# lachinov/brats2019

Hardware: AMD Instinct MI355X
Metric: volumes_per_sec_fwd_bwd_128cubed_x4ch (higher is better)
Workload: dtype bf16

## Files before the change

brats2019_amd/csrc/pointwise.hip:

```cpp
#include "pw_helpers.hpp"
#include "augment_voxel.hpp"

namespace ru {

template <int VEC, int COT>
__global__ __launch_bounds__(256) void conv1_kernel(const Conv1Args a) {
    const int n = blockIdx.z;
    const int co0 = blockIdx.y * COT;
    const size_t V = a.V;
    const size_t v = ((size_t)blockIdx.x * 256 + threadIdx.x) * VEC;
    if (v >= V) return;
    float acc[COT][VEC];
#pragma unroll
    for (int o = 0; o < COT; ++o)
#pragma unroll
        for (int k = 0; k < VEC; ++k) acc[o][k] = 0.f;
    int widx[COT];
#pragma unroll
    for (int o = 0; o < COT; ++o) widx[o] = (co0 + o < a.Cout) ? co0 + o : a.Cout - 1;

    const float* xp = a.x0 + (size_t)n * a.C0 * V + v;
    const float* wr = a.wT;
#pragma unroll 4
    for (int c = 0; c < a.C0; ++c) {
// ... 466 lines not shown
        if (dbeta) dbeta[g * cpg + j] = (float)db;
    }
}
int gn_bwd_finalize_launch(const float* partials, int nblk, const float* gamma, const float* mean, const float* rstd,
                           float* coef, float* dgamma, float* dbeta, int N, int C, size_t V, int G, hipStream_t s, int s2_sign) {
    RU_REQUIRE(C % G == 0 && C / G <= 256, "groupnorm: C must be divisible by G (and C/G <= 256)");
    const size_t shm = (size_t)N * (C / G) * 2 * sizeof(double);
    RU_REQUIRE(shm <= 60000, "groupnorm backward: batch x channels-per-group too large for the finalize kernel");
    if (nblk > 32) hipLaunchKernelGGL(gn_bwd_finalize_kernel<64>, dim3(G), dim3(N * (C / G) > 4 ? 512 : 256), shm, s, partials, nblk, gamma, mean, rstd, coef, dgamma, dbeta, N, C, V, G, s2_sign);
    else if (nblk > 4) hipLaunchKernelGGL(gn_bwd_finalize_kernel<16>, dim3(G), dim3(256), shm, s, partials, nblk, gamma, mean, rstd, coef, dgamma, dbeta, N, C, V, G, s2_sign);
    else hipLaunchKernelGGL(gn_bwd_finalize_kernel<4>, dim3(G), dim3(256), shm, s, partials, nblk, gamma, mean, rstd, coef, dgamma, dbeta, N, C, V, G, s2_sign);
    RU_CHECK_LAUNCH("gn_bwd_finalize_kernel");
    return RU_OK;
}

template <int VEC>
__global__ __launch_bounds__(256) void gn_bwd_apply_kernel(const float* __restrict__ x, const float* __restrict__ dy, const float* __restrict__ scale,
                                                           const float* __restrict__ shift, const float* __restrict__ coef, float slope,
                                                           float* __restrict__ dx, size_t V) {
    const size_t row = blockIdx.y;
    const float a = scale[row], b = shift[row];
    const float cA = coef[row * 3], cB = coef[row * 3 + 1], cC = coef[row * 3 + 2];
    const size_t base = row * V;
    for (size_t v = ((size_t)blockIdx.x * 256 + threadIdx.x) * VEC; v < V; v += (size_t)gridDim.x * 256 * VEC) {
        if (VEC == 4) {
            const float4 t = *reinterpret_cast<const float4*>(x + base + v);
            const float4 d = *reinterpret_cast<const float4*>(dy + base + v);
            float4 o;
            o.x = cA * ((t.x * a + b) > 0.f ? d.x : d.x * slope) + (cB * t.x + cC);
            o.y = cA * ((t.y * a + b) > 0.f ? d.y : d.y * slope) + (cB * t.y + cC);
            o.z = cA * ((t.z * a + b) > 0.f ? d.z : d.z * slope) + (cB * t.z + cC);
            o.w = cA * ((t.w * a + b) > 0.f ? d.w : d.w * slope) + (cB * t.w + cC);
            *reinterpret_cast<float4*>(dx + base + v) = o;
        } else {
            const float t = x[base + v], d = dy[base + v];
            dx[base + v] = cA * ((t * a + b) > 0.f ? d : d * slope) + (cB * t + cC);
        }
    }
}
int gn_bwd_apply_launch(const float* x, const float* dy, const float* scale, const float* shift, const float* coef,
                        float slope, float* dx, int N, int C, size_t V, hipStream_t s) {
    if (V % 4 == 0) hipLaunchKernelGGL(gn_bwd_apply_kernel<4>, rows_grid(V, 4, N * C), dim3(256), 0, s, x, dy, scale, shift, coef, slope, dx, V);
    else hipLaunchKernelGGL(gn_bwd_apply_kernel<1>, rows_grid(V, 1, N * C), dim3(256), 0, s, x, dy, scale, shift, coef, slope, dx, V);
    RU_CHECK_LAUNCH("gn_bwd_apply_kernel");
    return RU_OK;
}

enum { EW_LRELU = 0, EW_LRELU_BWD = 1, EW_SIGMOID = 2, EW_SIGMOID_BWD = 3, EW_ADD = 4, EW_FILL = 5 };
template <int OP>
__global__ __launch_bounds__(256) void ew_kernel(const float* __restrict__ a, const float* __restrict__ b, float* __restrict__ y, size_t n, float p) {
    const size_t stride = (size_t)gridDim.x * 256;
    for (size_t i = (size_t)blockIdx.x * 256 + threadIdx.x; i < n; i += stride) {
        float r;
        if (OP == EW_LRELU) r = lrelu(a[i], p);
        else if (OP == EW_LRELU_BWD) r = a[i] > 0.f ? b[i] : b[i] * p;
        else if (OP == EW_SIGMOID) r = 1.f / (1.f + expf(-a[i]));
        else if (OP == EW_SIGMOID_BWD) { const float q = a[i]; r = b[i] * q * (1.f - q); }
        else if (OP == EW_ADD) r = a[i] + b[i];
        else r = p;
        y[i] = r;
    }
}
template <int OP>
static int ew_launch(const float* a, const float* b, float* y, size_t n, float p, hipStream_t s, const char* name) {
    if (n == 0) return RU_OK;
    hipLaunchKernelGGL(ew_kernel<OP>, dim3(grid1d(n, 256 * 4, 8192)), dim3(256), 0, s, a, b, y, n, p);
    RU_CHECK_LAUNCH(name);
    return RU_OK;
}
int lrelu_fwd_launch(const float* x, float* y, size_t n, float slope, hipStream_t s) { return ew_launch<EW_LRELU>(x, nullptr, y, n, slope, s, "lrelu"); }
int lrelu_bwd_launch(const float* yv, const float* dy, float* dx, size_t n, float slope, hipStream_t s) { return ew_launch<EW_LRELU_BWD>(yv, dy, dx, n, slope, s, "lrelu_bwd"); }
int sigmoid_launch(const float* x, float* y, size_t n, hipStream_t s) { return ew_launch<EW_SIGMOID>(x, nullptr, y, n, 0.f, s, "sigmoid"); }
int sigmoid_bwd_launch(const float* p, const float* dp, float* dz, size_t n, hipStream_t s) { return ew_launch<EW_SIGMOID_BWD>(p, dp, dz, n, 0.f, s, "sigmoid_bwd"); }
int add_launch(const float* a, const float* b, float* y, size_t n, hipStream_t s) { return ew_launch<EW_ADD>(a, b, y, n, 0.f, s, "add"); }
__global__ __launch_bounds__(256) void sum_partials_kernel(const float* __restrict__ part, int ksplit, size_t n, float* __restrict__ y) {
    const size_t n4 = n >> 2;
    for (size_t i = (size_t)blockIdx.x * 256 + threadIdx.x; i < n4; i += (size_t)gridDim.x * 256) {
        float4 acc = reinterpret_cast<const float4*>(part)[i];
        for (int z = 1; z < ksplit; ++z) {
            const float4 t = reinterpret_cast<const float4*>(part + (size_t)z * n)[i];
            acc.x += t.x; acc.y += t.y; acc.z += t.z; acc.w += t.w;
        }
        reinterpret_cast<float4*>(y)[i] = acc;
    }
    if (blockIdx.x == 0 && threadIdx.x < (n & 3)) {
        const size_t i = (n4 << 2) + threadIdx.x;
        float acc = part[i];
        for (int z = 1; z < ksplit; ++z) acc += part[(size_t)z * n + i];
        y[i] = acc;
    }
}
int sum_partials_launch(const float* part, int ksplit, size_t n, float* y, hipStream_t s) {
    RU_REQUIRE(part && y && ksplit >= 1, "sum_partials: bad argument");
    RU_REQUIRE(ksplit == 1 || (n & 3) == 0, "sum_partials: partial tensors of %zu floats are not 16-byte aligned to each other", n);
    hipLaunchKernelGGL(sum_partials_kernel, dim3(grid1d(n, 256 * 4, 2048)), dim3(256), 0, s, part, ksplit, n, y);
    RU_CHECK_LAUNCH("sum_partials_kernel");
    return RU_OK;
}
int fill_launch(float* p, float v, size_t n, hipStream_t s) { return ew_launch<EW_FILL>(nullptr, nullptr, p, n, v, s, "fill"); }

__global__ __launch_bounds__(256) void up2_fwd_kernel(const float* __restrict__ x, float* __restrict__ y, int NC, int D, int H, int W) {
    const int Do = 2 * D, Ho = 2 * H;
    const size_t total = (size_t)NC * Do * Ho * W;
    for (size_t i = (size_t)blockIdx.x * 256 + threadIdx.x; i < total; i += (size_t)gridDim.x * 256) {
        const int k = (int)(i % W);
        size_t r = i / W;
        const int yo = (int)(r % Ho); r /= Ho;
        const int zo = (int)(r % Do);
        const size_t nc = r / Do;
        int z0, z1, y0, y1; float lz0, lz1, ly0, ly1;
        up2_src(zo, D, z0, z1, lz0, lz1);
        up2_src(yo, H, y0, y1, ly0, ly1);
        const int km = k > 0 ? k - 1 : 0, kp = k < W - 1 ? k + 1 : k;
        const float* p00 = x + ((nc * D + z0) * H + y0) * (size_t)W;
        const float* p01 = x + ((nc * D + z0) * H + y1) * (size_t)W;
        const float* p10 = x + ((nc * D + z1) * H + y0) * (size_t)W;
        const float* p11 = x + ((nc * D + z1) * H + y1) * (size_t)W;
        const float e0 = k > 0 ? 0.25f : 1.f, e1 = k > 0 ? 0.75f : 0.f;
        const int ei0 = k > 0 ? km : 0, ei1 = k > 0 ? k : (W > 1 ? 1 : 0);
        const float ev = lz0 * (ly0 * (e0 * p00[ei0] + e1 * p00[ei1]) + ly1 * (e0 * p01[ei0] + e1 * p01[ei1])) +
                         lz1 * (ly0 * (e0 * p10[ei0] + e1 * p10[ei1]) + ly1 * (e0 * p11[ei0] + e1 * p11[ei1]));
        const float ov = lz0 * (ly0 * (0.75f * p00[k] + 0.25f * p00[kp]) + ly1 * (0.75f * p01[k] + 0.25f * p01[kp])) +
                         lz1 * (ly0 * (0.75f * p10[k] + 0.25f * p10[kp]) + ly1 * (0.75f * p11[k] + 0.25f * p11[kp]));
        float* yp = y + ((nc * Do + zo) * Ho + yo) * (size_t)(2 * W) + 2 * k;
        *reinterpret_cast<float2*>(yp) = make_float2(ev, ov);
    }
}
__global__ __launch_bounds__(256) void up2_fwd_vec_kernel(const float* __restrict__ x, float* __restrict__ y, int NC, int D, int H, int W) {
    const int Do = 2 * D, Ho = 2 * H, Wh = W / 2;
    const size_t total = (size_t)NC * Do * Ho * Wh;
    for (size_t i = (size_t)blockIdx.x * 256 + threadIdx.x; i < total; i += (size_t)gridDim.x * 256) {
        const int m = (int)(i % Wh);
        size_t r = i / Wh;
        const int yo = (int)(r % Ho); r /= Ho;
        const int zo = (int)(r % Do);
        const size_t nc = r / Do;
        int z0, z1, y0, y1; float lz0, lz1, ly0, ly1;
        up2_src(zo, D, z0, z1, lz0, lz1);
        up2_src(yo, H, y0, y1, ly0, ly1);
        const int k = 2 * m;
        const int km = k > 0 ? k - 1 : 0, kpp = k + 2 < W ? k + 2 : W - 1;
        const float* rows[4] = {x + ((nc * D + z0) * H + y0) * (size_t)W, x + ((nc * D + z0) * H + y1) * (size_t)W,
                                x + ((nc * D + z1) * H + y0) * (size_t)W, x + ((nc * D + z1) * H + y1) * (size_t)W};
        const float wgt[4] = {lz0 * ly0, lz0 * ly1, lz1 * ly0, lz1 * ly1};
        float o[4];
        float rowv[4][4];
#pragma unroll
        for (int q = 0; q < 4; ++q) {
            const float a0 = rows[q][km], a1 = rows[q][k], a2 = rows[q][k + 1], a3 = rows[q][kpp];
            rowv[q][0] = k > 0 ? 0.25f * a0 + 0.75f * a1 : 1.f * a1 + 0.f * a2;
            rowv[q][1] = 0.75f * a1 + 0.25f * a2;
            rowv[q][2] = 0.25f * a1 + 0.75f * a2;
            rowv[q][3] = 0.75f * a2 + 0.25f * a3;
        }
        (void)wgt;
#pragma unroll
        for (int t = 0; t < 4; ++t)
            o[t] = lz0 * (ly0 * rowv[0][t] + ly1 * rowv[1][t]) + lz1 * (ly0 * rowv[2][t] + ly1 * rowv[3][t]);
        *reinterpret_cast<float4*>(y + ((nc * Do + zo) * Ho + yo) * (size_t)(2 * W) + 4 * m) = make_float4(o[0], o[1], o[2], o[3]);
    }
}
int up2_fwd_launch(const float* x, float* y, int N, int C, int D, int H, int W, hipStream_t s) {
    if ((W & 1) == 0) {
        const size_t total = (size_t)N * C * 2 * D * 2 * H * (W / 2);
        hipLaunchKernelGGL(up2_fwd_vec_kernel, dim3(grid1d(total, 256)), dim3(256), 0, s, x, y, N * C, D, H, W);
        RU_CHECK_LAUNCH("up2_fwd_vec_kernel");
        return RU_OK;
    }
    const size_t total = (size_t)N * C * 2 * D * 2 * H * W;
    hipLaunchKernelGGL(up2_fwd_kernel, dim3(grid1d(total, 256)), dim3(256), 0, s, x, y, N * C, D, H, W);
    RU_CHECK_LAUNCH("up2_fwd_kernel");
    return RU_OK;
}

__global__ __launch_bounds__(256) void up2_bwd_kernel(const float* __restrict__ dy, float* __restrict__ dx, int NC, int D, int H, int W) {
    const int Do = 2 * D, Ho = 2 * H, Wo = 2 * W;
    const size_t total = (size_t)NC * D * H * W;
    for (size_t i = (size_t)blockIdx.x * 256 + threadIdx.x; i < total; i += (size_t)gridDim.x * 256) {
        const int kx = (int)(i % W);
        size_t r = i / W;
        const int ky = (int)(r % H); r /= H;
        const int kz = (int)(r % D);
        const size_t nc = r / D;
        float wz[4], wy[4], wx[4];
#pragma unroll
        for (int t = 0; t < 4; ++t) {
            const int oz = 2 * kz - 1 + t, oy = 2 * ky - 1 + t, ox = 2 * kx - 1 + t;
            wz[t] = (oz >= 0 && oz < Do) ? up2_coef(oz, D, kz) : 0.f;
            wy[t] = (oy >= 0 && oy < Ho) ? up2_coef(oy, H, ky) : 0.f;
            wx[t] = (ox >= 0 && ox < Wo) ? up2_coef(ox, W, kx) : 0.f;
        }
        float acc = 0.f;
#pragma unroll
        for (int a = 0; a < 4; ++a) {
            if (wz[a] == 0.f) continue;
            const int oz = 2 * kz - 1 + a;
            float accy = 0.f;
#pragma unroll
            for (int b = 0; b < 4; ++b) {
                if (wy[b] == 0.f) continue;
                const int oy = 2 * ky - 1 + b;
                const float* p = dy + ((nc * Do + oz) * Ho + oy) * (size_t)Wo;
                float accx = 0.f;
#pragma unroll
                for (int c = 0; c < 4; ++c) {
                    const int ox = 2 * kx - 1 + c;
                    if (wx[c] != 0.f) accx += wx[c] * p[ox];
                }
                accy += wy[b] * accx;
            }
            acc += wz[a] * accy;
        }
        dx[i] = acc;
    }
}
__global__ __launch_bounds__(256) void up2_bwd_vec_kernel(const float* __restrict__ dy, float* __restrict__ dx, int NC, int D, int H, int W) {
    const int Do = 2 * D, Ho = 2 * H, Wo = 2 * W, Wh = W / 2;
    const size_t total = (size_t)NC * D * H * Wh;
    for (size_t i = (size_t)blockIdx.x * 256 + threadIdx.x; i < total; i += (size_t)gridDim.x * 256) {
        const int m = (int)(i % Wh);
        size_t r = i / Wh;
        const int ky = (int)(r % H); r /= H;
        const int kz = (int)(r % D);
        const size_t nc = r / D;
        const int k0 = 2 * m, k1 = 2 * m + 1;
        float wz[4], wy[4], wa[4], wb[4];
#pragma unroll
        for (int t = 0; t < 4; ++t) {
            const int oz = 2 * kz - 1 + t, oy = 2 * ky - 1 + t, oa = 2 * k0 - 1 + t, ob = 2 * k1 - 1 + t;
            wz[t] = (oz >= 0 && oz < Do) ? up2_coef(oz, D, kz) : 0.f;
            wy[t] = (oy >= 0 && oy < Ho) ? up2_coef(oy, H, ky) : 0.f;
            wa[t] = (oa >= 0 && oa < Wo) ? up2_coef(oa, W, k0) : 0.f;
            wb[t] = (ob >= 0 && ob < Wo) ? up2_coef(ob, W, k1) : 0.f;
        }
        const int oxl = 4 * m - 1 >= 0 ? 4 * m - 1 : 0, oxr = 4 * m + 4 < Wo ? 4 * m + 4 : Wo - 1;
        float acc0 = 0.f, acc1 = 0.f;
#pragma unroll
        for (int a = 0; a < 4; ++a) {
            const int oz = 2 * kz - 1 + a;
            const int ozc = oz < 0 ? 0 : (oz >= Do ? Do - 1 : oz);
            float ay0 = 0.f, ay1 = 0.f;
#pragma unroll
            for (int b = 0; b < 4; ++b) {
                const int oy = 2 * ky - 1 + b;
                const int oyc = oy < 0 ? 0 : (oy >= Ho ? Ho - 1 : oy);
                const float* p = dy + ((nc * Do + ozc) * Ho + oyc) * (size_t)Wo;
                const float4 f = *reinterpret_cast<const float4*>(p + 4 * m);
                const float fl = p[oxl], fr = p[oxr];
                ay0 += wy[b] * (wa[0] * fl + wa[1] * f.x + wa[2] * f.y + wa[3] * f.z);
                ay1 += wy[b] * (wb[0] * f.y + wb[1] * f.z + wb[2] * f.w + wb[3] * fr);
            }
            acc0 += wz[a] * ay0;
            acc1 += wz[a] * ay1;
        }
        *reinterpret_cast<float2*>(dx + ((nc * D + kz) * H + ky) * (size_t)W + 2 * m) = make_float2(acc0, acc1);
    }
}
int up2_bwd_launch(const float* dy, float* dx, int N, int C, int D, int H, int W, hipStream_t s) {
    if ((W & 1) == 0) {
        const size_t tv = (size_t)N * C * D * H * (W / 2);
        hipLaunchKernelGGL(up2_bwd_vec_kernel, dim3(grid1d(tv, 256)), dim3(256), 0, s, dy, dx, N * C, D, H, W);
        RU_CHECK_LAUNCH("up2_bwd_vec_kernel");
        return RU_OK;
    }
    const size_t total = (size_t)N * C * D * H * W;
    hipLaunchKernelGGL(up2_bwd_kernel, dim3(grid1d(total, 256)), dim3(256), 0, s, dy, dx, N * C, D, H, W);
    RU_CHECK_LAUNCH("up2_bwd_kernel");
    return RU_OK;
}

constexpr int BG_CHUNK = 16384;
size_t bias_grad_workspace_bytes(int N, int C, size_t V) { return (size_t)N * C * ((V + BG_CHUNK - 1) / BG_CHUNK) * sizeof(float); }
__global__ __launch_bounds__(256) void bias_partial_kernel(const float* __restrict__ dy, float* __restrict__ part, size_t V, int nblk) {
    __shared__ float buf[4];
    const size_t row = blockIdx.y;
    const size_t v0 = (size_t)blockIdx.x * BG_CHUNK;
    const size_t v1 = v0 + BG_CHUNK < V ? v0 + BG_CHUNK : V;
    float s1 = 0.f;
    for (size_t v = v0 + threadIdx.x; v < v1; v += 256) s1 += dy[row * V + v];
    s1 = block_sum(s1, buf);
    if (threadIdx.x == 0) part[row * nblk + blockIdx.x] = s1;
}
__global__ __launch_bounds__(256) void bias_final_kernel(const float* __restrict__ part, float* __restrict__ db, int N, int C, int nblk) {
    __shared__ double buf[4];
    const int c = blockIdx.x;
    double s1 = 0.0;
    for (int i = threadIdx.x; i < N * nblk; i += 256) {
        const int n = i / nblk, b = i % nblk;
        s1 += (double)part[((size_t)n * C + c) * nblk + b];
    }
    s1 = block_sum_d(s1, buf);
    if (threadIdx.x == 0) db[c] = (float)s1;
}
int bias_grad_launch(const float* dy, float* db, int N, int C, size_t V, void* ws, size_t ws_bytes, hipStream_t s) {
    if (!ws || ws_bytes < bias_grad_workspace_bytes(N, C, V)) { set_error("bias_grad: workspace too small"); return RU_ENOMEM; }
    const int nblk = (int)((V + BG_CHUNK - 1) / BG_CHUNK);
    hipLaunchKernelGGL(bias_partial_kernel, dim3(nblk, N * C), dim3(256), 0, s, dy, (float*)ws, V, nblk);
    RU_CHECK_LAUNCH("bias_partial_kernel");
    hipLaunchKernelGGL(bias_final_kernel, dim3(C), dim3(256), 0, s, (const float*)ws, db, N, C, nblk);
    RU_CHECK_LAUNCH("bias_final_kernel");
    return RU_OK;
}

template <bool CRIT>
__global__ __launch_bounds__(256) void head_grad_c4_kernel(const float* __restrict__ p, const float* __restrict__ dp, float* __restrict__ d4,
                                                           float* __restrict__ part, int C, size_t V, int nblk, const CritGradArgs cg) {
    __shared__ float buf[4];
    const size_t n = blockIdx.y;
    const size_t v0 = (size_t)blockIdx.x * BG_CHUNK;
    const size_t v1 = v0 + BG_CHUNK < V ? v0 + BG_CHUNK : V;
    const float* pp = p + n * C * V;
    const float* dpp = dp + n * C * V;
    float4* op = reinterpret_cast<float4*>(d4) + n * V;
    float sum[4] = {0.f, 0.f, 0.f, 0.f};
    float kg[4] = {0.f, 0.f, 0.f, 0.f}, kp[4] = {0.f, 0.f, 0.f, 0.f}, cb = 0.f;
    const float one_eps = (float)(1.0 + 1e-6);
    if constexpr (CRIT) {
        for (int c = 0; c < C && c < 4; ++c) {
            const double I = cg.sums[c] + 1e-6, U = cg.sums[C + c] + 2e-6;
            const double k = (double)cg.priority * (2.0 / (double)C) * (double)cg.w_dice;
            kg[c] = (float)(-k / U);
            kp[c] = (float)(2.0 * k * I / (U * U));
        }
        cb = (float)((double)cg.w_bce / cg.count);
    }
    for (size_t v = v0 + (size_t)threadIdx.x * 4; v < v1; v += 1024) {
        float d[4][4];
#pragma unroll
        for (int c = 0; c < 4; ++c) {
            const bool ok = c < C;
            const float4 q = *reinterpret_cast<const float4*>(pp + (ok ? c : 0) * V + v);
            float4 g = *reinterpret_cast<const float4*>(dpp + (ok ? c : 0) * V + v);
            if constexpr (CRIT) {
                const float pv[4] = {q.x, q.y, q.z, q.w}, gv[4] = {g.x, g.y, g.z, g.w};
                float o[4];
#pragma unroll
                for (int e = 0; e < 4; ++e) o[e] = crit_grad_value(pv[e], gv[e], kg[c], kp[c], cb, cg.bgw, one_eps);
                g = make_float4(o[0], o[1], o[2], o[3]);
            }
            d[c][0] = ok ? g.x * q.x * (1.f - q.x) : 0.f;
            d[c][1] = ok ? g.y * q.y * (1.f - q.y) : 0.f;
            d[c][2] = ok ? g.z * q.z * (1.f - q.z) : 0.f;
            d[c][3] = ok ? g.w * q.w * (1.f - q.w) : 0.f;
            sum[c] += (d[c][0] + d[c][1]) + (d[c][2] + d[c][3]);
        }
#pragma unroll
        for (int e = 0; e < 4; ++e) op[v + e] = make_float4(d[0][e], d[1][e], d[2][e], d[3][e]);
    }
#pragma unroll
    for (int c = 0; c < 4; ++c) {
        const float t = block_sum(sum[c], buf);
        if (threadIdx.x == 0 && c < C) part[(n * C + c) * nblk + blockIdx.x] = t;
    }
}
int head_grad_c4_launch(const float* p, const float* dp, float* d4, float* db, int N, int C, size_t V, void* ws, size_t ws_bytes, hipStream_t s) {
    RU_REQUIRE(C > 0 && C <= 4 && V % 4 == 0, "head_grad_c4: 1..4 channels, V %% 4 == 0");
    if (!ws || ws_bytes < bias_grad_workspace_bytes(N, C, V)) { set_error("head_grad_c4: workspace too small"); return RU_ENOMEM; }
    const int nblk = (int)((V + BG_CHUNK - 1) / BG_CHUNK);
    hipLaunchKernelGGL(head_grad_c4_kernel<false>, dim3(nblk, N), dim3(256), 0, s, p, dp, d4, (float*)ws, C, V, nblk, CritGradArgs{});
    RU_CHECK_LAUNCH("head_grad_c4_kernel");
    hipLaunchKernelGGL(bias_final_kernel, dim3(C), dim3(256), 0, s, (const float*)ws, db, N, C, nblk);
    RU_CHECK_LAUNCH("bias_final_kernel");
    return RU_OK;
}
int head_grad_c4_crit_launch(const float* p, const CritGradArgs& cg, float* d4, float* db, int N, int C, size_t V, void* ws, size_t ws_bytes, hipStream_t s) {
    RU_REQUIRE(C > 0 && C <= 4 && V % 4 == 0 && cg.target && cg.sums, "head_grad_c4_crit: 1..4 channels, V %% 4 == 0, target and sums");
    if (!ws || ws_bytes < bias_grad_workspace_bytes(N, C, V)) { set_error("head_grad_c4_crit: workspace too small"); return RU_ENOMEM; }
    const int nblk = (int)((V + BG_CHUNK - 1) / BG_CHUNK);
    hipLaunchKernelGGL(head_grad_c4_kernel<true>, dim3(nblk, N), dim3(256), 0, s, p, cg.target, d4, (float*)ws, C, V, nblk, cg);
    RU_CHECK_LAUNCH("head_grad_c4_kernel<crit>");
    hipLaunchKernelGGL(bias_final_kernel, dim3(C), dim3(256), 0, s, (const float*)ws, db, N, C, nblk);
    RU_CHECK_LAUNCH("bias_final_kernel");
    return RU_OK;
}

constexpr int CR_CHUNK = 8192;
int crit_tiles(size_t V) { return (int)((V + CR_CHUNK - 1) / CR_CHUNK); }
__global__ __launch_bounds__(256) void crit_partial_kernel(const float* __restrict__ p, const float* __restrict__ g, float* __restrict__ part,
                                                           size_t V, int nblk, float bgw) {
    __shared__ float buf[4];
    const size_t row = blockIdx.y;
    const size_t v0 = (size_t)blockIdx.x * CR_CHUNK;
    const size_t v1 = v0 + CR_CHUNK < V ? v0 + CR_CHUNK : V;
    const float one_eps = (float)(1.0 + 1e-6);
    float si = 0.f, su = 0.f, sb = 0.f;
    for (size_t v = v0 + threadIdx.x; v < v1; v += 256) {
        const float pv = p[row * V + v], gv = g[row * V + v];
        si += pv * gv;
        su += pv * pv + gv;
        sb += gv * logf(pv + 1e-6f) + bgw * (1.f - gv) * logf(one_eps - pv);
    }
    si = block_sum(si, buf);
    su = block_sum(su, buf);
    sb = block_sum(sb, buf);
    if (threadIdx.x == 0) {
        float* q = part + (row * nblk + blockIdx.x) * 3;
        q[0] = si; q[1] = su; q[2] = sb;
    }
}
__global__ __launch_bounds__(256) void crit_final_kernel(const float* __restrict__ part, double* __restrict__ sums, int N, int C, int nblk) {
    __shared__ double buf[4];
    double bce = 0.0;
    for (int c = 0; c < C; ++c) {
        double si = 0.0, su = 0.0, sb = 0.0;
        for (int i = threadIdx.x; i < N * nblk; i += 256) {
            const int n = i / nblk, b = i % nblk;
            const float* q = part + (((size_t)n * C + c) * nblk + b) * 3;
            si += (double)q[0]; su += (double)q[1]; sb += (double)q[2];
        }
        si = block_sum_d(si, buf);
        su = block_sum_d(su, buf);
        sb = block_sum_d(sb, buf);
        if (threadIdx.x == 0) { sums[c] = si; sums[C + c] = su; }
        bce += sb;
    }
    if (threadIdx.x == 0) sums[2 * C] = bce;
}
int crit_sums_launch(const float* p, const float* g, double* sums, int N, int C, size_t V, float bgw, void* ws, size_t ws_bytes, hipStream_t s) {
    const int nblk = crit_tiles(V);
    if (!ws || ws_bytes < (size_t)N * C * nblk * 3 * sizeof(float)) { set_error("criterion: workspace too small"); return RU_ENOMEM; }
    hipLaunchKernelGGL(crit_partial_kernel, dim3(nblk, N * C), dim3(256), 0, s, p, g, (float*)ws, V, nblk, bgw);
    RU_CHECK_LAUNCH("crit_partial_kernel");
    hipLaunchKernelGGL(crit_final_kernel, dim3(1), dim3(256), 0, s, (const float*)ws, sums, N, C, nblk);
    RU_CHECK_LAUNCH("crit_final_kernel");
    return RU_OK;
}
__global__ void crit_value_kernel(const double* __restrict__ sums, int C, double count, double priority, double w_dice, double w_bce,
                                  double* __restrict__ out) {
    double q = threadIdx.x < (unsigned)C ? 2.0 * (sums[threadIdx.x] + 1e-6) / (sums[C + threadIdx.x] + 2e-6) : 0.0;
    for (int o = 32; o > 0; o >>= 1) q += __shfl_xor(q, o);
    if (threadIdx.x == 0) {
        const double dice = priority * (1.0 - q / C), bce = -sums[2 * C] / count;
        out[0] = w_dice * dice + w_bce * bce; out[1] = dice; out[2] = bce;
    }
}
int crit_value_launch(const double* sums, int C, double count, double priority, double w_dice, double w_bce, double* out3, hipStream_t s) {
    hipLaunchKernelGGL(crit_value_kernel, dim3(1), dim3(64), 0, s, sums, C, count, priority, w_dice, w_bce, out3);
    RU_CHECK_LAUNCH("crit_value_kernel");
    return RU_OK;
}
__global__ __launch_bounds__(256) void crit_grad_kernel(const float* __restrict__ p, const float* __restrict__ g, const double* __restrict__ sums,
                                                        double count, float w_dice, float w_bce, float bgw, float priority,
                                                        float* __restrict__ dp, int C, size_t V) {
    const size_t row = blockIdx.y;
    const int c = (int)(row % C);
    const double I = sums[c] + 1e-6, U = sums[C + c] + 2e-6;
    const double k = (double)priority * (2.0 / (double)C) * (double)w_dice;
    const float cg = (float)(-k / U), cp = (float)(2.0 * k * I / (U * U));
    const float cb = (float)((double)w_bce / count);
    const float one_eps = (float)(1.0 + 1e-6);
    for (size_t v = (size_t)blockIdx.x * 256 + threadIdx.x; v < V; v += (size_t)gridDim.x * 256) {
        const float pv = p[row * V + v], gv = g[row * V + v];
        dp[row * V + v] = crit_grad_value(pv, gv, cg, cp, cb, bgw, one_eps);
    }
}
int crit_grad_launch(const float* p, const float* g, const double* sums, double count, float w_dice, float w_bce,
                     float bgw, float priority, float* dp, int N, int C, size_t V, hipStream_t s) {
    hipLaunchKernelGGL(crit_grad_kernel, rows_grid(V, 1, N * C), dim3(256), 0, s, p, g, sums, count, w_dice, w_bce, bgw, priority, dp, C, V);
    RU_CHECK_LAUNCH("crit_grad_kernel");
    return RU_OK;
}

__global__ __launch_bounds__(256) void tta_merge_kernel(const float* __restrict__ p, int K, unsigned flips, float* __restrict__ mean_out,
                                                        unsigned char* __restrict__ mask_out, unsigned long long* __restrict__ counts,
                                                        int C, int D, int H, int W) {
    __shared__ unsigned int cnt[4];
    const size_t V = (size_t)D * H * W;
    const int c = blockIdx.y;
    if (threadIdx.x < 4) cnt[threadIdx.x] = 0;
    __syncthreads();
    unsigned int local = 0;
    for (size_t v = (size_t)blockIdx.x * 256 + threadIdx.x; v < V; v += (size_t)gridDim.x * 256) {
        const int x = (int)(v % W);
        const int y = (int)((v / W) % H);
        const int z = (int)(v / ((size_t)W * H));
        float acc = 0.f;
        for (int k = 0; k < K; ++k) {
            const unsigned f = (flips >> (3 * k)) & 7u;
            const int zz = (f & 1u) ? D - 1 - z : z, yy = (f & 2u) ? H - 1 - y : y, xx = (f & 4u) ? W - 1 - x : x;
            const float t = p[(((size_t)k * C + c) * D + zz) * H * W + (size_t)yy * W + xx];
            acc = k == 0 ? t : acc + t;
        }
        const float m = acc / (float)K;
        if (mean_out) mean_out[(size_t)c * V + v] = m;
        const bool on = m > 0.5f;
        mask_out[(size_t)c * V + v] = on ? 1 : 0;
        local += on ? 1u : 0u;
    }
    atomicAdd(&cnt[threadIdx.x >> 6], local);
    __syncthreads();
    if (threadIdx.x == 0) atomicAdd(&counts[c], (unsigned long long)cnt[0] + cnt[1] + cnt[2] + cnt[3]);
}
__global__ __launch_bounds__(256) void compose_labels_kernel(const unsigned char* __restrict__ mask, const unsigned long long* __restrict__ counts,
                                                             unsigned long long et_min, unsigned char* __restrict__ labels, size_t V) {
    const bool et_on = counts[2] > et_min;
    for (size_t v = (size_t)blockIdx.x * 256 + threadIdx.x; v < V; v += (size_t)gridDim.x * 256) {
        unsigned char l = 0;
        if (mask[v]) l = 2;
        if (mask[V + v]) l = 1;
        if (et_on && mask[2 * V + v]) l = 4;
        labels[v] = l;
    }
}
int tta_merge_launch(const float* p, int K, unsigned flips, float* mean_out, unsigned char* mask, unsigned long long* counts, int C, int D, int H, int W, hipStream_t s) {
    RU_REQUIRE(K >= 1 && K <= 8 && C >= 1, "tta_merge: 1..8 predictions");
    hipError_t e = hipMemsetAsync(counts, 0, sizeof(unsigned long long) * C, s);
    if (e != hipSuccess) return hip_fail(e, "hipMemsetAsync(counts)");
    const size_t V = (size_t)D * H * W;
    hipLaunchKernelGGL(tta_merge_kernel, dim3(grid1d(V, 256 * 8, 512), C), dim3(256), 0, s, p, K, flips, mean_out, mask, counts, C, D, H, W);
    RU_CHECK_LAUNCH("tta_merge_kernel");
    return RU_OK;
}
int compose_labels_launch(const unsigned char* mask, const unsigned long long* counts, unsigned long long et_min, unsigned char* labels, size_t V, hipStream_t s) {
    hipLaunchKernelGGL(compose_labels_kernel, dim3(grid1d(V, 256, 4096)), dim3(256), 0, s, mask, counts, et_min, labels, V);
    RU_CHECK_LAUNCH("compose_labels_kernel");
    return RU_OK;
}

__global__ __launch_bounds__(256) void layout_convert_kernel(const float* __restrict__ src, float* __restrict__ dst, int CB, size_t V, int to_c16) {
    __shared__ float tile[16][65];
    const size_t v0 = (size_t)blockIdx.x * 64;
    const size_t nb = blockIdx.y;
    const int t = threadIdx.x;
    const float* s_nc = src + nb * 16 * V;
    float* d_nc = dst + nb * 16 * V;
    if (to_c16) {
#pragma unroll
        for (int j = 0; j < 4; ++j) {
            const int c = (t >> 6) + 4 * j, v = t & 63;
            tile[c][v] = v0 + v < V ? s_nc[(size_t)c * V + v0 + v] : 0.f;
        }
        __syncthreads();
#pragma unroll
        for (int j = 0; j < 4; ++j) {
            const int e = t + 256 * j, v = e >> 4, c = e & 15;
            if (v0 + v < V) d_nc[(v0 + v) * 16 + c] = tile[c][v];
        }
    } else {
#pragma unroll
        for (int j = 0; j < 4; ++j) {
            const int e = t + 256 * j, v = e >> 4, c = e & 15;
            tile[c][v] = v0 + v < V ? s_nc[(v0 + v) * 16 + c] : 0.f;
        }
        __syncthreads();
#pragma unroll
        for (int j = 0; j < 4; ++j) {
            const int c = (t >> 6) + 4 * j, v = t & 63;
            if (v0 + v < V) d_nc[(size_t)c * V + v0 + v] = tile[c][v];
        }
    }
}
int layout_convert_launch(const float* src, float* dst, int N, int C, size_t V, int to_c16, hipStream_t s) {
    RU_REQUIRE(C > 0 && C % 16 == 0, "layout_convert: C must be a multiple of 16");
    hipLaunchKernelGGL(layout_convert_kernel, dim3((unsigned)((V + 63) / 64), (unsigned)(N * (C / 16))), dim3(256), 0, s, src, dst, C / 16, V, to_c16);
    RU_CHECK_LAUNCH("layout_convert_kernel");
    return RU_OK;
}

__global__ __launch_bounds__(256) void pad_to_c16_kernel(const float* __restrict__ src, float* __restrict__ dst, int C, size_t V) {
    const size_t n = blockIdx.y;
    const float* sp = src + n * C * V;
    float4* dp = reinterpret_cast<float4*>(dst + n * 16 * V);
    for (size_t f = (size_t)blockIdx.x * 256 + threadIdx.x; f < V * 4; f += (size_t)gridDim.x * 256) {
        const size_t v = f >> 2;
        const int c0 = (int)(f & 3) * 4;
        float4 o;
        o.x = c0 + 0 < C ? sp[(size_t)(c0 + 0) * V + v] : 0.f;
        o.y = c0 + 1 < C ? sp[(size_t)(c0 + 1) * V + v] : 0.f;
        o.z = c0 + 2 < C ? sp[(size_t)(c0 + 2) * V + v] : 0.f;
        o.w = c0 + 3 < C ? sp[(size_t)(c0 + 3) * V + v] : 0.f;
        dp[f] = o;
    }
}
int pad_to_c16_launch(const float* src, float* dst, int N, int C, size_t V, hipStream_t s) {
    RU_REQUIRE(C > 0 && C <= 16, "pad_to_c16: 1..16 channels");
    hipLaunchKernelGGL(pad_to_c16_kernel, dim3(grid1d(V * 4, 256, 4096), (unsigned)N), dim3(256), 0, s, src, dst, C, V);
    RU_CHECK_LAUNCH("pad_to_c16_kernel");
    return RU_OK;
}

__global__ __launch_bounds__(256) void pad_to_c4_kernel(const float* __restrict__ src, float* __restrict__ dst, int C, size_t V) {
    const size_t n = blockIdx.y;
    const float* sp = src + n * C * V;
    float4* dp = reinterpret_cast<float4*>(dst) + n * V;
    for (size_t v = (size_t)blockIdx.x * 256 + threadIdx.x; v < V; v += (size_t)gridDim.x * 256) {
        float4 o;
        o.x = sp[v];
        o.y = C > 1 ? sp[V + v] : 0.f;
        o.z = C > 2 ? sp[2 * V + v] : 0.f;
        o.w = C > 3 ? sp[3 * V + v] : 0.f;
        dp[v] = o;
    }
}
int pad_to_c4_launch(const float* src, float* dst, int N, int C, size_t V, hipStream_t s) {
    RU_REQUIRE(C > 0 && C <= 4, "pad_to_c4: 1..4 channels");
    hipLaunchKernelGGL(pad_to_c4_kernel, dim3(grid1d(V, 256, 4096), (unsigned)N), dim3(256), 0, s, src, dst, C, V);
    RU_CHECK_LAUNCH("pad_to_c4_kernel");
    return RU_OK;
}

__global__ __launch_bounds__(256) void dice_counts_kernel(const float* __restrict__ p, const float* __restrict__ g,
                                                          unsigned long long* __restrict__ counts, size_t V) {
    __shared__ unsigned int sm[4][2];
    const size_t row = blockIdx.y;
    const float* pp = p + row * V;
    const float* gp = g + row * V;
    unsigned int inter = 0, uni = 0;
    if ((V & 3) == 0) {
        const size_t V4 = V >> 2;
        for (size_t v = (size_t)blockIdx.x * 256 + threadIdx.x; v < V4; v += (size_t)gridDim.x * 256) {
            const float4 a = reinterpret_cast<const float4*>(pp)[v], b = reinterpret_cast<const float4*>(gp)[v];
            const bool a0 = a.x > 0.5f, a1 = a.y > 0.5f, a2 = a.z > 0.5f, a3 = a.w > 0.5f;
            const bool b0 = b.x > 0.5f, b1 = b.y > 0.5f, b2 = b.z > 0.5f, b3 = b.w > 0.5f;
            inter += (unsigned)(a0 && b0) + (unsigned)(a1 && b1) + (unsigned)(a2 && b2) + (unsigned)(a3 && b3);
            uni += (unsigned)a0 + (unsigned)a1 + (unsigned)a2 + (unsigned)a3 + (unsigned)b0 + (unsigned)b1 + (unsigned)b2 + (unsigned)b3;
        }
    } else {
        for (size_t v = (size_t)blockIdx.x * 256 + threadIdx.x; v < V; v += (size_t)gridDim.x * 256) {
            const bool a = pp[v] > 0.5f, b = gp[v] > 0.5f;
            inter += (a && b) ? 1u : 0u;
            uni += (a ? 1u : 0u) + (b ? 1u : 0u);
        }
    }
#pragma unroll
    for (int o = 32; o > 0; o >>= 1) { inter += __shfl_xor(inter, o); uni += __shfl_xor(uni, o); }
    if ((threadIdx.x & 63) == 0) { sm[threadIdx.x >> 6][0] = inter; sm[threadIdx.x >> 6][1] = uni; }
    __syncthreads();
    if (threadIdx.x == 0) {
        atomicAdd(&counts[row * 2], (unsigned long long)sm[0][0] + sm[1][0] + sm[2][0] + sm[3][0]);
        atomicAdd(&counts[row * 2 + 1], (unsigned long long)sm[0][1] + sm[1][1] + sm[2][1] + sm[3][1]);
    }
}
int dice_counts_launch(const float* p, const float* g, unsigned long long* counts, int rows, size_t V, hipStream_t s) {
    hipError_t e = hipMemsetAsync(counts, 0, sizeof(unsigned long long) * 2 * rows, s);
    if (e != hipSuccess) return hip_fail(e, "hipMemsetAsync(dice counts)");
    hipLaunchKernelGGL(dice_counts_kernel, dim3(grid1d(V, 256 * 4 * 8, 64), rows), dim3(256), 0, s, p, g, counts, V);
    RU_CHECK_LAUNCH("dice_counts_kernel");
    return RU_OK;
}

__global__ void dice_accumulate_kernel(const unsigned long long* __restrict__ counts, double* __restrict__ acc, int N, int C, int nacc) {
    const int c = threadIdx.x;
    if (c >= nacc) return;
    double sum = 0.0;
    for (int n = 0; n < N; ++n) {
        const float num = (float)counts[((size_t)n * C + c) * 2], den = (float)counts[((size_t)n * C + c) * 2 + 1];
        float r = 2.f * num / den;
        if (r != r) r = 1.f;
        sum += (double)r;
    }
    acc[c] += sum / (double)N;
}
int dice_accumulate_launch(const unsigned long long* counts, double* acc, int N, int C, int nacc, hipStream_t s) {
    RU_REQUIRE(counts && acc && N > 0 && nacc > 0 && nacc <= C && nacc <= 64, "dice_accumulate: bad argument");
    hipLaunchKernelGGL(dice_accumulate_kernel, dim3(1), dim3(64), 0, s, counts, acc, N, C, nacc);
    RU_CHECK_LAUNCH("dice_accumulate_kernel");
    return RU_OK;
}

constexpr int ZS_CHUNK = 16384;
size_t zscore_workspace_bytes(int C, size_t V) { return (size_t)C * ((V + ZS_CHUNK - 1) / ZS_CHUNK) * 3 * sizeof(double); }
__global__ __launch_bounds__(256) void zscore_partial_kernel(const float* __restrict__ x, double* __restrict__ part, size_t V, int nblk) {
    __shared__ double buf[4];
    const size_t c = blockIdx.y;
    const size_t v0 = (size_t)blockIdx.x * ZS_CHUNK, v1 = v0 + ZS_CHUNK < V ? v0 + ZS_CHUNK : V;
    double n = 0.0, s1 = 0.0, s2 = 0.0;
    for (size_t v = v0 + threadIdx.x; v < v1; v += 256) {
        const double t = (double)x[c * V + v];
        n += t > 0.0 ? 1.0 : 0.0;
        s1 += t;
        s2 += t * t;
    }
// ... 74 lines not shown
```

Baseline: 271.9.

## Software-pipeline head gradient loads and coalesce float4 stores through LDS

Rewrites the head-gradient kernel to prefetch two iterations ahead with a rotating three-stage register buffer, so global loads overlap computation. Interleaved float4 outputs now go through a per-wavefront LDS exchange buffer, making the stores to d4 contiguous across lanes instead of strided by four. It also specializes the kernel on C==4 versus C<=3 to drop the unused channel's loads. The cost is more registers, 16KB of shared memory per block and wave-level barriers, which may lower occupancy.

```diff
diff --git a/brats2019_amd/csrc/pointwise.hip b/brats2019_amd/csrc/pointwise.hip
--- a/brats2019_amd/csrc/pointwise.hip
+++ b/brats2019_amd/csrc/pointwise.hip
@@ -792,10 +792,11 @@
     return RU_OK;
 }
 
-template <bool CRIT>
+template <bool CRIT, bool FOUR>
 __global__ __launch_bounds__(256) void head_grad_c4_kernel(const float* __restrict__ p, const float* __restrict__ dp, float* __restrict__ d4,
                                                            float* __restrict__ part, int C, size_t V, int nblk, const CritGradArgs cg) {
     __shared__ float buf[4];
+    __shared__ float4 xch[1024];
     const size_t n = blockIdx.y;
     const size_t v0 = (size_t)blockIdx.x * BG_CHUNK;
     const size_t v1 = v0 + BG_CHUNK < V ? v0 + BG_CHUNK : V;
@@ -814,28 +815,69 @@
         }
         cb = (float)((double)cg.w_bce / cg.count);
     }
-    for (size_t v = v0 + (size_t)threadIdx.x * 4; v < v1; v += 1024) {
-        float d[4][4];
-#pragma unroll
-        for (int c = 0; c < 4; ++c) {
-            const bool ok = c < C;
-            const float4 q = *reinterpret_cast<const float4*>(pp + (ok ? c : 0) * V + v);
-            float4 g = *reinterpret_cast<const float4*>(dpp + (ok ? c : 0) * V + v);
-            if constexpr (CRIT) {
-                const float pv[4] = {q.x, q.y, q.z, q.w}, gv[4] = {g.x, g.y, g.z, g.w};
-                float o[4];
-#pragma unroll
-                for (int e = 0; e < 4; ++e) o[e] = crit_grad_value(pv[e], gv[e], kg[c], kp[c], cb, cg.bgw, one_eps);
-                g = make_float4(o[0], o[1], o[2], o[3]);
+    constexpr int NC = FOUR ? 4 : 3;
+    float4 qa[NC], ga[NC], qb[NC], gb[NC], qc[NC], gc[NC];
+    auto fetch = [&](size_t v, float4 (&q)[NC], float4 (&g)[NC]) __attribute__((always_inline)) {
+#pragma unroll
+        for (int c = 0; c < NC; ++c) {
+            const size_t o = (size_t)(c < C ? c : 0) * V + v;
+            q[c] = *reinterpret_cast<const float4*>(pp + o);
+            g[c] = *reinterpret_cast<const float4*>(dpp + o);
+        }
+    };
+    const int wbase = (threadIdx.x >> 6) * 256, lane = threadIdx.x & 63;
+    auto convert = [&](int r, bool live, const float4 (&qq)[NC], const float4 (&gg)[NC]) __attribute__((always_inline)) {
+        if (live) {
+            float d[4][4] = {};
+#pragma unroll
+            for (int c = 0; c < NC; ++c) {
+                const bool ok = c < C;
+                const float4 q = qq[c];
+                float4 g = gg[c];
+                if constexpr (CRIT) {
+                    const float pv[4] = {q.x, q.y, q.z, q.w}, gv[4] = {g.x, g.y, g.z, g.w};
+                    float o[4];
+#pragma unroll
+                    for (int e = 0; e < 4; ++e) o[e] = crit_grad_value(pv[e], gv[e], kg[c], kp[c], cb, cg.bgw, one_eps);
+                    g = make_float4(o[0], o[1], o[2], o[3]);
+                }
+                d[c][0] = ok ? g.x * q.x * (1.f - q.x) : 0.f;
+                d[c][1] = ok ? g.y * q.y * (1.f - q.y) : 0.f;
+                d[c][2] = ok ? g.z * q.z * (1.f - q.z) : 0.f;
+                d[c][3] = ok ? g.w * q.w * (1.f - q.w) : 0.f;
+                sum[c] += (d[c][0] + d[c][1]) + (d[c][2] + d[c][3]);
             }
-            d[c][0] = ok ? g.x * q.x * (1.f - q.x) : 0.f;
-            d[c][1] = ok ? g.y * q.y * (1.f - q.y) : 0.f;
-            d[c][2] = ok ? g.z * q.z * (1.f - q.z) : 0.f;
-            d[c][3] = ok ? g.w * q.w * (1.f - q.w) : 0.f;
-            sum[c] += (d[c][0] + d[c][1]) + (d[c][2] + d[c][3]);
-        }
-#pragma unroll
-        for (int e = 0; e < 4; ++e) op[v + e] = make_float4(d[0][e], d[1][e], d[2][e], d[3][e]);
+#pragma unroll
+            for (int e = 0; e < 4; ++e) xch[wbase + 4 * lane + e] = make_float4(d[0][e], d[1][e], d[2][e], d[3][e]);
+        }
+        __builtin_amdgcn_fence(__ATOMIC_RELEASE, "wavefront");
+        __builtin_amdgcn_wave_barrier();
+        __builtin_amdgcn_fence(__ATOMIC_ACQUIRE, "wavefront");
+        const size_t vw = v0 + (size_t)r * 1024 + wbase;
+#pragma unroll
+        for (int k = 0; k < 4; ++k) {
+            const size_t v = vw + k * 64 + lane;
+            if (v < v1) op[v] = xch[wbase + k * 64 + lane];
+        }
+        __builtin_amdgcn_fence(__ATOMIC_RELEASE, "wavefront");
+        __builtin_amdgcn_wave_barrier();
+    };
+    const size_t vt = v0 + (size_t)threadIdx.x * 4;
+    const int nr = vt < v1 ? (int)((v1 - vt + 1023) / 1024) : 0;
+    const int nrb = (int)((v1 - v0 + 1023) / 1024);
+    auto at = [&](int r) { return nr > 0 ? vt + (size_t)(r < nr ? r : nr - 1) * 1024 : v0; };
+    fetch(at(0), qa, ga);
+    fetch(at(1), qb, gb);
+    for (int r = 0;; r += 3) {
+        fetch(at(r + 2), qc, gc);
+        convert(r, r < nr, qa, ga);
+        if (r + 1 >= nrb) break;
+        fetch(at(r + 3), qa, ga);
+        convert(r + 1, r + 1 < nr, qb, gb);
+        if (r + 2 >= nrb) break;
+        fetch(at(r + 4), qb, gb);
+        convert(r + 2, r + 2 < nr, qc, gc);
+        if (r + 3 >= nrb) break;
     }
 #pragma unroll
     for (int c = 0; c < 4; ++c) {
@@ -847,7 +889,8 @@
     RU_REQUIRE(C > 0 && C <= 4 && V % 4 == 0, "head_grad_c4: 1..4 channels, V %% 4 == 0");
     if (!ws || ws_bytes < bias_grad_workspace_bytes(N, C, V)) { set_error("head_grad_c4: workspace too small"); return RU_ENOMEM; }
     const int nblk = (int)((V + BG_CHUNK - 1) / BG_CHUNK);
-    hipLaunchKernelGGL(head_grad_c4_kernel<false>, dim3(nblk, N), dim3(256), 0, s, p, dp, d4, (float*)ws, C, V, nblk, CritGradArgs{});
+    if (C == 4) hipLaunchKernelGGL((head_grad_c4_kernel<false, true>), dim3(nblk, N), dim3(256), 0, s, p, dp, d4, (float*)ws, C, V, nblk, CritGradArgs{});
+    else hipLaunchKernelGGL((head_grad_c4_kernel<false, false>), dim3(nblk, N), dim3(256), 0, s, p, dp, d4, (float*)ws, C, V, nblk, CritGradArgs{});
     RU_CHECK_LAUNCH("head_grad_c4_kernel");
     hipLaunchKernelGGL(bias_final_kernel, dim3(C), dim3(256), 0, s, (const float*)ws, db, N, C, nblk);
     RU_CHECK_LAUNCH("bias_final_kernel");
@@ -857,7 +900,8 @@
     RU_REQUIRE(C > 0 && C <= 4 && V % 4 == 0 && cg.target && cg.sums, "head_grad_c4_crit: 1..4 channels, V %% 4 == 0, target and sums");
     if (!ws || ws_bytes < bias_grad_workspace_bytes(N, C, V)) { set_error("head_grad_c4_crit: workspace too small"); return RU_ENOMEM; }
     const int nblk = (int)((V + BG_CHUNK - 1) / BG_CHUNK);
-    hipLaunchKernelGGL(head_grad_c4_kernel<true>, dim3(nblk, N), dim3(256), 0, s, p, cg.target, d4, (float*)ws, C, V, nblk, cg);
+    if (C == 4) hipLaunchKernelGGL((head_grad_c4_kernel<true, true>), dim3(nblk, N), dim3(256), 0, s, p, cg.target, d4, (float*)ws, C, V, nblk, cg);
+    else hipLaunchKernelGGL((head_grad_c4_kernel<true, false>), dim3(nblk, N), dim3(256), 0, s, p, cg.target, d4, (float*)ws, C, V, nblk, cg);
     RU_CHECK_LAUNCH("head_grad_c4_kernel<crit>");
     hipLaunchKernelGGL(bias_final_kernel, dim3(C), dim3(256), 0, s, (const float*)ws, db, N, C, nblk);
     RU_CHECK_LAUNCH("bias_final_kernel");
```

After: 272.0, median of 4. About the same (+0.0%).
